# mache102/HashNeRF-pytorch

Hardware: AMD Instinct MI355X
Metric: training rays/sec (fwd+bwd) on chair; PSNR@5k iters (higher is better)
Workload: dtype fp32 (MLP GEMMs split-bf16 MFMA: 3 parts fwd, 2 parts grads); 1 GPU; chair 1xMI355X N_rand=4096 64+128 L16 F2 T19 finest512 (BASELINE configs[1]); rays_per_gpu=4096, global_batch=4096, samples_per_ray=64+128, log2_hashmap_size=19, finest_res=512, parallelism=dp1

## Files before the change

hashnerf-pytorch_amd/_lib.py:

```python
from __future__ import annotations

import ctypes as C
import os
from typing import Optional

import torch

HERE = os.path.dirname(os.path.abspath(__file__))
LIB_PATH = os.environ.get("HN_LIB_PATH") or os.path.join(HERE, "lib", "libhashnerf_amd.so")
MAX_LEVELS = 32
ABI_VERSION = 14
RENDER_FEAT_PER_RAY = 9728
MLP_PARAMS = 9344
MLP_PACKED_FLOATS = 30208

_lib = None


class HnGrid(C.Structure):
    _fields_ = [("n_levels", C.c_int32), ("n_features", C.c_int32),
                ("log2_hashmap_size", C.c_int32), ("reserved", C.c_int32),
                ("box_min", C.c_float * 3), ("box_max", C.c_float * 3),
                ("grid_size", (C.c_float * 3) * MAX_LEVELS)]

# ... 96 lines not shown
                ("g_raw_f", _P), ("d_table", _P), ("d_coarse", HnMlpGrad), ("d_fine", HnMlpGrad),
                ("table_step", C.POINTER(HnRadamTensor)), ("tv", C.c_void_p), ("g_tv", _P),
                ("table_live", _P), ("table_live_levels", C.c_int32), ("owner_defer", C.c_int32),
                ("loss", C.POINTER(HnRenderLoss)), ("mlp_step", C.POINTER(HnRadamTensor)),
                ("repack", C.c_int32), ("prepass_done", C.c_int32), ("next_batch", C.POINTER(HnNextBatch))]


class HnTvArgs(C.Structure):
    _fields_ = [("n_levels", C.c_int32), ("log2_hashmap_size", C.c_int32),
                ("cube", C.c_int32 * MAX_LEVELS), ("min_vertex", _P), ("table", _P)]


RADAM_MAX_TENSORS = 16


class HnRayPool(C.Structure):
    _fields_ = [("n_images", C.c_int32), ("H", C.c_int32), ("W", C.c_int32), ("pose_stride", C.c_int32),
                ("fx", C.c_double), ("fy", C.c_double), ("cx", C.c_double), ("cy", C.c_double),
                ("near", C.c_float), ("far", C.c_float), ("seed", C.c_uint64)]


POOL_ORDER_MAX = 8192

SIGNATURES = {
    "hn_abi_version": (C.c_int32, []),
    "hn_status_string": (C.c_char_p, [C.c_int32]),
    "hn_device_faults": (C.c_int32, [C.POINTER(C.c_int32), C.c_int32]),
    "hn_encode_fwd": (C.c_int32, [C.POINTER(HnGrid), _P, C.c_int64, _P, _P, _P, _P]),
    "hn_encode_bwd": (C.c_int32, [C.POINTER(HnGrid), _P, C.c_int64, _P, _P, _P]),
    "hn_sh_fwd": (C.c_int32, [_P, C.c_int64, _P, _P]),
    "hn_encode_bwd_input": (C.c_int32, [C.POINTER(HnGrid), _P, C.c_int64, _P, _P, _P, _P]),
    "hn_sh_bwd": (C.c_int32, [_P, _P, C.c_int64, _P, _P]),
    "hn_mlp_workspace_bytes": (C.c_size_t, []),
    "hn_mlp_fwd": (C.c_int32, [C.POINTER(HnMlp), _P, C.c_int64, _P, _P, C.c_size_t, _P]),
    "hn_mlp_bwd": (C.c_int32, [C.POINTER(HnMlp), _P, _P, C.c_int64, _P, C.POINTER(HnMlpGrad), _P,
                               C.c_size_t, _P]),
    "hn_composite_fwd": (C.c_int32, [_P, _P, _P, _P, C.c_int64, C.c_int32, C.c_int32, _P, _P, _P,
                                     _P, _P, _P, _P]),
    "hn_composite_bwd": (C.c_int32, [_P, _P, _P, _P, C.c_int64, C.c_int32, C.c_int32, _P, _P, _P,
                                     _P, _P, _P, _P]),
    "hn_composite_bwd_inputs": (C.c_int32, [_P, _P, _P, _P, C.c_int64, C.c_int32, C.c_int32, _P, _P, _P,
                                            _P, _P, _P, _P, _P]),
    "hn_sample_pdf": (C.c_int32, [_P, _P, _P, C.c_int64, C.c_int32, C.c_int32, _P, _P]),
    "hn_tv_fwd": (C.c_int32, [C.POINTER(HnTvArgs), _P, _P]),
    "hn_tv_bwd": (C.c_int32, [C.POINTER(HnTvArgs), _P, _P, _P]),
    "hn_radam_step": (C.c_int32, [C.POINTER(HnRadamTensor), C.c_int32, _P]),
    "hn_sample_rays": (C.c_int32, [C.POINTER(HnRaySampler), _P, _P, C.c_int64, _P, _P, _P]),
    "hn_sample_rays_morton_workspace_bytes": (C.c_size_t, [C.POINTER(HnRaySampler)]),
    "hn_uniform_philox": (C.c_int32, [C.c_uint64, C.POINTER(HnUniformDraw), C.c_int32, _P]),
    "hn_sample_batch_morton": (C.c_int32, [C.POINTER(HnRaySampler), _P, _P, C.c_int64, _P, _P, _P, C.c_size_t,
                                           C.c_uint64, C.POINTER(HnUniformDraw), C.c_int32, _P]),
    "hn_sample_rays_morton": (C.c_int32, [C.POINTER(HnRaySampler), _P, _P, C.c_int64, _P, _P, _P, C.c_size_t,
                                          _P]),
    "hn_sample_pool": (C.c_int32, [C.POINTER(HnRayPool), _P, _P, _P, C.c_int64, C.c_int64, _P, _P, _P]),
    "hn_sample_pool_ordered": (C.c_int32, [C.POINTER(HnRayPool), _P, _P, _P, C.c_int64, C.c_int64,
                                           C.POINTER(C.c_float), C.POINTER(C.c_float), _P, _P, _P, C.c_uint64,
                                           C.POINTER(HnUniformDraw), C.c_int32, _P]),
    "hn_sample_rays_ndc": (C.c_int32, [C.POINTER(HnRaySampler), _P, _P, C.c_int64, _P, _P, C.POINTER(HnRayNdc), _P]),
    "hn_sample_rays_morton_ndc": (C.c_int32, [C.POINTER(HnRaySampler), _P, _P, C.c_int64, _P, _P, _P, C.c_size_t,
                                              C.POINTER(HnRayNdc), _P]),
    "hn_sample_batch_morton_ndc": (C.c_int32, [C.POINTER(HnRaySampler), _P, _P, C.c_int64, _P, _P, _P, C.c_size_t,
                                               C.c_uint64, C.POINTER(HnUniformDraw), C.c_int32,
                                               C.POINTER(HnRayNdc), _P]),
    "hn_sample_pool_ndc": (C.c_int32, [C.POINTER(HnRayPool), _P, _P, _P, C.c_int64, C.c_int64, _P, _P,
                                       C.POINTER(HnRayNdc), _P]),
    "hn_sample_pool_ordered_ndc": (C.c_int32, [C.POINTER(HnRayPool), _P, _P, _P, C.c_int64, C.c_int64,
                                               C.POINTER(C.c_float), C.POINTER(C.c_float), _P, _P, _P, C.c_uint64,
                                               C.POINTER(HnUniformDraw), C.c_int32, C.POINTER(HnRayNdc), _P]),
    "hn_blender_images": (C.c_int32, [_P, C.c_int64, C.c_int32, C.c_int32, C.c_int32, C.c_int32, _P, _P]),
    "hn_loss_fwd": (C.c_int32, [_P, _P, _P, _P, _P, C.c_int64, _P, C.c_int32, C.c_float, C.c_float,
                                C.c_float, _P, _P]),
    "hn_loss_bwd": (C.c_int32, [_P, _P, _P, C.c_int64, C.c_int32, C.c_float, C.c_float, C.c_float, _P,
                                _P, _P, _P, _P, _P, _P]),
    "hn_loss_fwd_bwd": (C.c_int32, [_P, _P, _P, _P, _P, C.c_int64, _P, C.c_int32, C.c_float, C.c_float,
                                    C.c_float, _P, _P, _P, _P, _P, _P, _P, _P]),
    "hn_render_workspace_bytes": (C.c_size_t, [C.POINTER(HnRenderCfg), C.c_int64]),
    "hn_render_scatter_mode": (C.c_int32, [C.POINTER(HnRenderCfg), C.c_int64]),
    "hn_render_fwd": (C.c_int32, [C.POINTER(HnRenderCfg), C.POINTER(HnRenderFwdArgs), _P,
                                  C.c_size_t, _P]),
    "hn_render_fwd_form": (C.c_int32, [C.POINTER(HnRenderCfg), C.POINTER(HnRenderFwdArgs), C.c_int32, _P,
                                       C.c_size_t, _P]),
    "hn_render_fwd_pick": (C.c_int32, [C.c_int64, C.POINTER(C.c_int32)]),
    "hn_render_fwd_deal": (C.c_int32, [C.c_int64, C.c_int64, _P, _P]),
    "hn_render_bwd": (C.c_int32, [C.POINTER(HnRenderCfg), C.POINTER(HnRenderBwdArgs), _P,
                                  C.c_size_t, _P]),
    "hn_render_bwd_ndc": (C.c_int32, [C.POINTER(HnRenderCfg), C.POINTER(HnRenderBwdArgs), _P, C.c_size_t,
                                      C.POINTER(HnRayNdc), _P]),
    "hn_render_bwd_rays_workspace_bytes": (C.c_size_t, [C.POINTER(HnRenderCfg), C.c_int64]),
    "hn_render_bwd_rays": (C.c_int32, [C.POINTER(HnRenderCfg), C.POINTER(HnRenderBwdArgs), _P, C.c_size_t, _P, _P]),
    "hn_render_image_workspace_bytes": (C.c_size_t, [C.POINTER(HnRenderCfg)]),
    "hn_render_image": (C.c_int32, [C.POINTER(HnRenderCfg), C.POINTER(HnImageArgs), _P, C.c_size_t, _P]),
    "hn_render_image_variant": (C.c_int32, [C.POINTER(HnRenderCfg), C.POINTER(HnImageArgs), C.c_int32, _P,
                                            C.c_size_t, _P]),
    "hn_render_views_workspace_bytes": (C.c_size_t, [C.POINTER(HnRenderCfg)]),
    "hn_render_views": (C.c_int32, [C.POINTER(HnRenderCfg), C.POINTER(HnViewArgs), _P, C.c_size_t, _P]),
    "hn_render_bins": (C.c_int32, [C.POINTER(HnRenderCfg), C.c_int64, C.POINTER(C.c_int32)]),
    "hn_render_bwd_owner": (C.c_int32, [C.POINTER(HnRenderCfg), C.POINTER(HnRenderBwdArgs), _P,
                                        C.c_size_t, C.c_int32, C.c_int32, _P]),
}


def lib():
    global _lib
    if _lib is None:
        if not os.path.exists(LIB_PATH):
            raise RuntimeError(
                f"hashnerf_amd: HIP library not built ({LIB_PATH}); run "
                "`python -c 'import __graft_entry__ as g; g.build()'` -- there is no CPU fallback")
        L = C.CDLL(LIB_PATH)
        for name, (res, args) in SIGNATURES.items():
            fn = getattr(L, name)
            fn.restype = res
            fn.argtypes = args
        _lib = L
    return _lib


def check(status: int, what: str):
    if status != 0:
        msg = lib().hn_status_string(status).decode()
        raise RuntimeError(f"hashnerf_amd.{what} failed: {msg} (status {status})")


FAULT_BITS = {1: "ring slot wait", 2: "ring drain (tiles left unscattered)", 4: "coarse-grad flag wait",
              8: "dW buffer wait", 16: "binned-scatter overflow records exhausted",
              32: "non-finite (NaN / Inf) feature gradient or sample point in the binned scatter",
              64: "gradient on a table row pair the live mask marks dead (fused table step)",
              128: "prepass_done without a training forward of these rays on this workspace"}


def check_device_faults(clear: bool = True):
    w = C.c_int32(0)
    check(lib().hn_device_faults(C.byref(w), int(clear)), "device_faults")
    if w.value:
        what = ", ".join(v for k, v in FAULT_BITS.items() if w.value & k) or str(w.value)
        raise RuntimeError(f"hashnerf_amd: the render backward reported a fault ({what}); "
                           "the gradients of the launches since the last check are invalid")


def ptr(t: Optional[torch.Tensor]):
    return None if t is None else C.c_void_p(t.data_ptr())


def stream(device: torch.device):
    return C.c_void_p(torch.cuda.current_stream(device).cuda_stream)


def require_device(*tensors: torch.Tensor):
    for t in tensors:
        if t is None:
            continue
        if not t.is_cuda:
            raise RuntimeError("hashnerf_amd: tensors must live on a ROCm (HIP) device; "
                               "the reference CPU path is not part of this package")
        if t.dtype != torch.float32:
            raise TypeError(f"hashnerf_amd: expected float32, got {t.dtype}")


def contig(t: Optional[torch.Tensor]):
    return None if t is None else t.contiguous()


def make_grid(n_levels, n_features, log2T, box_min, box_max, grid_sizes) -> HnGrid:
    g = HnGrid()
    g.n_levels, g.n_features, g.log2_hashmap_size = int(n_levels), int(n_features), int(log2T)
    bmin = [float(v) for v in box_min]
# ... 23 lines not shown
```

hashnerf-pytorch_amd/csrc/hn_mlp.h:

```cpp
#pragma once
#include "hn_common.h"

namespace hn {

constexpr int kSplitF = 3;
constexpr int kSplitB = 2;
enum : int { R_F0, R_F1, R_F2G, R_F2S, R_F3, R_F4, R_B4, R_B3, R_B2G, R_B2S, R_B1, R_B0, R_N };
constexpr int kRegKS[R_N] = {16, 32, 8, 8, 32, 32, 4, 32, 32, 32, 8, 32};
constexpr int kRegOB[R_N] = {2, 1, 2, 2, 2, 1, 2, 2, 1, 1, 2, 1};
constexpr int kSplitFC = kSplitF;
constexpr int reg_ns(int r) {
  return kRegKS[r] % 8 ? 0 : (r < R_F2G ? kSplitF : (r < R_B4 ? kSplitFC : kSplitB));
}
constexpr int reg_gpo(int r) { return reg_ns(r) ? reg_ns(r) * kRegKS[r] / 8 : kRegKS[r] / 4; }
constexpr int reg_off(int r) {
  int o = 0;
  for (int i = 0; i < r; ++i) o += kRegOB[i] * reg_gpo(i) * 256;
  return o;
}
enum : int {
  G_F0 = reg_off(R_F0), G_F1 = reg_off(R_F1), G_F2G = reg_off(R_F2G), G_F2S = reg_off(R_F2S),
  G_F3 = reg_off(R_F3), G_F4 = reg_off(R_F4), G_B4 = reg_off(R_B4), G_B3 = reg_off(R_B3),
  G_B2G = reg_off(R_B2G), G_B2S = reg_off(R_B2S), G_B1 = reg_off(R_B1), G_B0 = reg_off(R_B0),
  G_END = reg_off(R_N)
};
static_assert(G_END <= HN_MLP_PACKED_FLOATS, "packed size");

enum : int { W_S0 = 0, W_S1 = 2048, W_C0 = 3072, W_C1 = 5056, W_C2 = 9152, W_END = 9344 };
static_assert(W_END == HN_MLP_PARAMS, "param count");

struct FragGlobal {
  static constexpr bool kRing = false;
  static constexpr int kLdsEnd = 0;
  const float* P;
  HN_DEV f32x4 operator()(int off, int lane) const { return frag_load(P, off, lane); }
};
struct FwdChunk {
  int r, ob, c;
};
constexpr FwdChunk kFwdSeq[] = {
    {R_F0, 0, 0}, {R_F0, 0, 1}, {R_F0, 1, 0}, {R_F0, 1, 1}, {R_F1, 0, 0}, {R_F1, 0, 1}, {R_F1, 0, 2},
    {R_F1, 0, 3}, {R_F2G, 0, 0}, {R_F2G, 1, 0}, {R_F3, 0, 0}, {R_F3, 0, 1}, {R_F3, 0, 2}, {R_F3, 0, 3},
    {R_F3, 1, 0}, {R_F3, 1, 1}, {R_F3, 1, 2}, {R_F3, 1, 3}, {R_F4, 0, 0}, {R_F4, 0, 1}, {R_F4, 0, 2},
    {R_F4, 0, 3}};
constexpr int kFwdSeqN = sizeof(kFwdSeq) / sizeof(kFwdSeq[0]);
constexpr int fwd_chunk_off(const FwdChunk& q) { return reg_off(q.r) + (q.ob * reg_gpo(q.r) + reg_ns(q.r) * q.c) * 256; }
constexpr int fwd_next_off(int r, int ob, int c) {
  for (int i = 0; i < kFwdSeqN; ++i)
    if (kFwdSeq[i].r == r && kFwdSeq[i].ob == ob && kFwdSeq[i].c == c) return fwd_chunk_off(kFwdSeq[(i + 1) % kFwdSeqN]);
  return -1;
}
struct FragRing {
  static constexpr bool kRing = true;
  static constexpr int kLdsEnd = 0;
  const float* P;
  float* slot;
  HN_DEV f32x4 operator()(int off, int lane) const { return frag_load(P, off, lane); }
};
constexpr int kFragResFloats = G_F2G;
struct FragRes {
  static constexpr bool kRing = false;
  static constexpr int kLdsEnd = kFragResFloats;
  const float* P;
  const float* res;
  HN_DEV f32x4 operator()(int off, int lane) const { return frag_load(P, off, lane); }
  HN_DEV f32x4 lds(int off, int lane) const { return *reinterpret_cast<const f32x4*>(res + off + 4 * lane); }
};
HN_DEV void ring_fill(const float* P, float* slot, int off, int lane) {
  int so = off * 4;
  asm volatile("" : "+s"(so));
  const __amdgpu_buffer_rsrc_t rs =
      __builtin_amdgcn_make_buffer_rsrc(const_cast<float*>(opaque_ptr(P)), (short)0, 0x7fffffff, 0x00020000);
#pragma unroll
  for (int q = 0; q < 3; ++q)
    __builtin_amdgcn_raw_ptr_buffer_load_lds(rs, (__attribute__((address_space(3))) void*)(slot + 256 * q), 16,
                                             lane * 16, so + 1024 * q, 0, 0);
}
HN_DEV void fwd_ring_start(const float* P, float* slot, int lane) {
  ring_fill(P, slot, fwd_chunk_off(kFwdSeq[0]), lane);
}
template <int R, typename BF, typename Src>
HN_DEV f32x16 gemm_src(const Src& src, int ob, f32x16 acc, int lane, BF bval);
template <int R, typename BF>
HN_DEV f32x16 gemm(const float* __restrict__ P, int ob, f32x16 acc, int lane, BF bval) {
  return gemm_src<R>(FragGlobal{P}, ob, acc, lane, bval);
}
template <int R, typename BF, typename Src>
HN_DEV f32x16 gemm_src(const Src& src, int ob, f32x16 acc, int lane, BF bval) {
  constexpr int KS = kRegKS[R], NS = reg_ns(R), GPO = reg_gpo(R), OFF = reg_off(R);
  auto ld = [&](int g) {
    if constexpr (OFF < Src::kLdsEnd) return src.lds(OFF + (ob * GPO + g) * 256, lane);
    else return src(OFF + (ob * GPO + g) * 256, lane);
  };
  if constexpr (NS > 0) {
#pragma unroll
    for (int c = 0; c < KS / 8; ++c) {
      SP<NS> a;
      if constexpr (Src::kRing && NS == 3) {
        asm volatile("s_waitcnt vmcnt(0)" ::: "memory");
#pragma unroll
        for (int q = 0; q < NS; ++q) a.p[q] = as_bf16x8(*reinterpret_cast<const f32x4*>(src.slot + 256 * q + 4 * lane));
        asm volatile("s_waitcnt lgkmcnt(0)" ::: "memory");
        ring_fill(src.P, src.slot, fwd_next_off(R, ob, c), lane);
      } else {
#pragma unroll
        for (int q = 0; q < NS; ++q) a.p[q] = as_bf16x8(ld(NS * c + q));
      }
      const SP<NS> b = splitn<NS>([&](int j) { return bval(8 * c + j); });
      acc = mfma_split<NS>(a, b, acc);
      __builtin_amdgcn_sched_barrier(0);
    }
    return acc;
  } else {
    f32x4 an = ld(0);
#pragma unroll
    for (int g = 0; g < KS / 4; ++g) {
      const f32x4 a = an;
      if (g + 1 < KS / 4) an = ld(g + 1);
#pragma unroll
      for (int j = 0; j < 4; ++j) acc = mfma(a[j], bval(4 * g + j), acc);
      __builtin_amdgcn_sched_barrier(0);
    }
    return acc;
  }
}

struct MlpAct {
  f32x16 h0[2];
  f32x16 s1;
  f32x16 c0[2];
  f32x16 c1[2];
  uint32_t m[3];
};
HN_DEV void relu_mask_or(const f32x16& v, uint32_t& m, int ob) {
  uint32_t w = 0u;
#pragma unroll
  for (int r = 15; r >= 0; --r) w = __builtin_amdgcn_alignbit(w, 0u - __float_as_uint(v[r]), 31u);
  m |= w << (16 * ob);
}

HN_DEV void relu16(f32x16& v) {
#pragma unroll
  for (int r = 0; r < 16; ++r) v[r] = __int_as_float(max(__float_as_int(v[r]), 0));
}
HN_DEV void mask16(f32x16& g, const f32x16& act) {
#pragma unroll
  for (int r = 0; r < 16; ++r) g[r] = act[r] > 0.f ? g[r] : 0.f;
}

struct NoLive {
  HN_DEV void operator()() const {}
};
template <bool MASKS = false, typename C0Init, typename Src, typename OnLive = NoLive>
HN_DEV void mlp_fwd_tile_src(const Src& P, const f32x16& feat, C0Init&& c0init, MlpAct& a, f32x16& c2,
                             int lane, bool skip_dead = false, OnLive&& on_live = OnLive{});
template <bool MASKS = false, typename C0Init>
HN_DEV void mlp_fwd_tile_c0(const float* __restrict__ P, const f32x16& feat, C0Init&& c0init,
                            MlpAct& a, f32x16& c2, int lane) {
  mlp_fwd_tile_src<MASKS>(FragGlobal{P}, feat, c0init, a, c2, lane);
}
template <bool MASKS, typename C0Init, typename Src, typename OnLive>
HN_DEV void mlp_fwd_tile_src(const Src& P, const f32x16& feat, C0Init&& c0init, MlpAct& a, f32x16& c2,
                             int lane, bool skip_dead, OnLive&& on_live) {
  a.m[0] = a.m[1] = a.m[2] = 0u;
#pragma unroll
  for (int ob = 0; ob < 2; ++ob) {
    a.h0[ob] = gemm_src<R_F0>(P, ob, zero16(), lane, [&](int s) { return feat[s]; });
    relu16(a.h0[ob]);
    if constexpr (MASKS) relu_mask_or(a.h0[ob], a.m[0], ob);
  }
  if constexpr (MASKS) asm volatile("" : "+v"(a.m[0]));
  a.s1 = gemm_src<R_F1>(P, 0, zero16(), lane, [&](int s) { return a.h0[s >> 4][s & 15]; });
  if (skip_dead && __ballot(lane < 32 && a.s1[0] > 0.f) == 0ull) {
    c2 = zero16();
    if constexpr (Src::kRing) {
      asm volatile("s_waitcnt vmcnt(0)" ::: "memory");
      ring_fill(P.P, P.slot, fwd_chunk_off(kFwdSeq[0]), lane);
    }
    return;
  }
  on_live();
#pragma unroll
  for (int ob = 0; ob < 2; ++ob) {
    f32x16 acc = c0init(ob);
    acc = gemm_src<R_F2G>(P, ob, acc, lane, [&](int s) { return a.s1[s]; });
    relu16(acc);
// ... 217 lines not shown
```

hashnerf-pytorch_amd/csrc/hn_render.hip:

```cpp
#include "hn_render_args.h"
#include "hn_render_fwd.h"
#include "hn_render_image.h"
#include "hn_mlp_bwd.h"
#include "hn_bwd_binned.h"
#include "hn_bwd_atomic.h"
#include "hn_bwd_rays.h"

#include <math.h>

#include <atomic>
#include <type_traits>

namespace hn {

__global__ __launch_bounds__(256) void render_comp_bwd_kernel(B1K k) {
  __shared__ float lds[kFwdWaves][kSf * 5];
  const int wave = __builtin_amdgcn_readfirstlane((int)threadIdx.x >> 6);
  const int lane = threadIdx.x & 63;
  if (k.bins && blockIdx.x == 0) zero_ovf_book(k);
  if (k.lout && blockIdx.x == 0) {
    loss_fwd_block<64 * kFwdWaves>(k.lrgb, k.lrgb0, k.ltarget, k.lsp, k.lsp0, k.B, k.ltv, k.n_tv, k.lworld,
                                   k.lsparse_w, k.ltv_w, k.lout);
    return;
  }
// ... 270 lines not shown
                          size_t ofs_c, size_t ofs_f, hipStream_t s, FieldK& f) {
  float *Pc = ws_at<float>(workspace, ofs_c), *Pf = ws_at<float>(workspace, ofs_f);
  if (int32_t st = weights_packed ? 0 : mlp_pack2_launch(&coarse, Pc, &fine, Pf, s)) return st;
  f = FieldK{make_grid_args(cfg->grid), cfg->white_bkgd, cfg->lindisp, t_vals, u, table, Pc, Pf};
  return HN_OK;
}

}

using namespace hn;

extern "C" size_t hn_render_workspace_bytes(const hn_render_cfg* cfg, int64_t n_rays) {
  return bwd_plan(cfg, n_rays).bytes();
}

extern "C" int32_t hn_render_scatter_mode(const hn_render_cfg* cfg, int64_t n_rays) {
  return bwd_mode(cfg, n_rays) == kModeSplit ? 2 : 1;
}

extern "C" int32_t hn_device_faults(int32_t* faults, int32_t clear) {
  if (!faults) return HN_E_NULL;
  int32_t st = hip_status(hipMemcpyFromSymbol(faults, HIP_SYMBOL(g_hn_fault), sizeof(int32_t)));
  if (st || !clear || *faults == 0) return st;
  const int32_t zero = 0;
  return hip_status(hipMemcpyToSymbol(HIP_SYMBOL(g_hn_fault), &zero, sizeof(int32_t)));
}

static int device_cus() {
  static std::atomic<int> cached[64];
  int dev = 0;
  if (hipGetDevice(&dev) != hipSuccess || dev < 0 || dev >= 64) return 0;
  int n = cached[dev].load(std::memory_order_relaxed);
  if (n == 0) {
    if (hipDeviceGetAttribute(&n, hipDeviceAttributeMultiprocessorCount, dev) != hipSuccess || n < 0) n = 0;
    cached[dev].store(n, std::memory_order_relaxed);
  }
  return n;
}
static int fwd_pick_form(int64_t n_rays, int cus) {
  return cus > 0 && (n_rays + kFwdResWaves - 1) / kFwdResWaves >= cus ? 2 : 1;
}
template <class F>
static void with_bool(bool b, F&& f) { b ? f(std::true_type{}) : f(std::false_type{}); }
static void launch_fwd(bool loss, bool ni64, bool res, int64_t n_rays, hipStream_t s, const RenderK& k) {
  const int bw = fwd_block_waves(res);
  const dim3 grid((unsigned)((n_rays + bw - 1) / bw)), block(64 * bw);
  with_bool(loss, [&](auto kLoss) {
    with_bool(ni64, [&](auto kNi64T) {
      with_bool(res, [&](auto kRes) {
        constexpr int ni = decltype(kNi64T)::value ? kNi64 : kNi;
        hipLaunchKernelGGL((render_fwd_kernel<decltype(kLoss)::value, ni, decltype(kRes)::value>), grid, block, 0, s,
                           k);
      });
    });
  });
}

extern "C" int32_t hn_render_fwd_pick(int64_t n_rays, int32_t* cus) {
  const int n = device_cus();
  if (cus) *cus = n;
  return fwd_pick_form(n_rays, n);
}

extern "C" int32_t hn_render_fwd_deal(int64_t n_rays, int64_t n_blocks, const uint8_t* run_key,
                                      int32_t* first_ray) {
  if (!first_ray) return HN_E_NULL;
  if (n_rays < 0 || n_blocks < 1 || n_blocks > (INT32_MAX / kFwdResWaves) || n_rays > n_blocks * kFwdResWaves)
    return HN_E_SHAPE;
  if (run_key)
    for (int64_t i = 0; i < n_blocks * kFwdResRuns; ++i)
      if (run_key[i] > kFwdResRunRays) return HN_E_SHAPE;
  for (int64_t b = 0; b < n_blocks; ++b) {
    const int x = (int)(b % kFwdResXcds);
    auto key_at = [&](int j) {
      const int64_t run = fwd_res_xcd_run(x, j);
      return run_key && run * kFwdResRunRays < n_rays ? (int)run_key[run] : 0;
    };
    for (int s = 0; s < kFwdResRuns; ++s)
      first_ray[b * kFwdResRuns + s] = (int32_t)(
          fwd_res_deal(n_blocks, b, s, [&](int nr, int pos) { return fwd_res_select(nr, pos, key_at); }) *
          kFwdResRunRays);
  }
  return HN_OK;
}

extern "C" int32_t hn_render_fwd(const hn_render_cfg* cfg, const hn_render_fwd_args* a,
                                 void* workspace, size_t ws_bytes, void* stream) {
  return hn_render_fwd_form(cfg, a, 0, workspace, ws_bytes, stream);
}

extern "C" int32_t hn_render_fwd_form(const hn_render_cfg* cfg, const hn_render_fwd_args* a, int32_t form,
                                      void* workspace, size_t ws_bytes, void* stream) {
  int32_t st = check_cfg(cfg);
  if (st) return st;
  if (form < 0 || form > 2) return HN_E_SHAPE;
  if (!a) return HN_E_NULL;
  if (a->n_rays < 0) return HN_E_SHAPE;
  if (a->n_rays == 0) return HN_OK;
  if (!a->rays || !a->t_vals || !a->u || !a->table || !mlp_ok(a->coarse) || !mlp_ok(a->fine))
    return HN_E_NULL;
  if (cfg->perturb && !a->t_rand) return HN_E_NULL;
  if (!a->rgb || !a->depth || !a->acc || !a->sparsity || !a->rgb0 || !a->depth0 || !a->acc0 ||
      !a->sparsity0 || !a->z_std || !a->z_coarse || !a->z_fine || !a->raw_c || !a->raw_f ||
      !a->fine_src)
    return HN_E_NULL;
  if (!workspace) return HN_E_NULL;
  const BwdPlan plan = bwd_plan(cfg, a->n_rays);
  if (ws_bytes < plan.bytes()) return HN_E_WORKSPACE;
  const bool ni64 = cfg->n_importance == kNi64;
  if (ni64 && a->feat && plan.mode != kModeSplit) return HN_E_SHAPE;
  if (a->loss) {
    if (!a->loss->target) return HN_E_NULL;
    if (!(a->loss->world > 0.f)) return HN_E_SHAPE;
    if (plan.mode != kModeSplit) return HN_E_SHAPE;
  }
  hipStream_t s = (hipStream_t)stream;
  RenderK k{};
  const WsLayout& L = plan.ws;
  if ((st = field_args(cfg, a->t_vals, a->u, a->table, a->coarse, a->fine, a->weights_packed, workspace, L.Pc, L.Pf,
                       s, k.f)))
    return st;
  k.perturb = cfg->perturb;
  k.B = a->n_rays;
  k.rays = a->rays; k.t_rand = a->t_rand;
  k.noise_c = a->noise_c; k.noise_f = a->noise_f;
  k.rgb = a->rgb; k.depth = a->depth; k.acc = a->acc; k.sparsity = a->sparsity;
  k.rgb0 = a->rgb0; k.depth0 = a->depth0; k.acc0 = a->acc0; k.sparsity0 = a->sparsity0;
  k.z_std = a->z_std; k.z_coarse = a->z_coarse; k.z_fine = a->z_fine;
  k.raw_c = a->raw_c; k.raw_f = a->raw_f; k.fine_src = a->fine_src; k.feat = a->feat;
  k.feat_nt = cfg->grid.log2_hashmap_size > 20;
  k.skip_dead = a->skip_dead_color != 0;
  const bool res = (form ? form : fwd_pick_form(a->n_rays, device_cus())) == 2;
  if (a->loss) {
    k.ltarget = a->loss->target;
    loss_factors(a->loss->world, a->loss->sparse_w, a->n_rays, k.lgm, k.lsparse);
    k.draw = ws_at<float>(workspace, L.draw);
    k.uflags = ws_at<uint8_t>(workspace, L.marks);
    k.stamp = ws_stamp(ws_at<int32_t>(workspace, L.lmeta));
  }
  launch_fwd(a->loss != nullptr, ni64, res, a->n_rays, s, k);
  return hip_status(hipGetLastError());
}

struct ImageWs {
  size_t Pc, Pf, slots, total;
};
static ImageWs image_ws_layout() {
  WsCursor c;
  ImageWs w;
  w.Pc = c.take(G_END);
  w.Pf = c.take(G_END);
  w.slots = c.take((size_t)kImgBlocks * kImgBlockWaves * kImgSlotFloats);
  w.total = c.at;
  return w;
}

extern "C" size_t hn_render_image_workspace_bytes(const hn_render_cfg* cfg) {
  return check_image_cfg(cfg) ? 0 : image_ws_layout().total * sizeof(float);
}
extern "C" size_t hn_render_views_workspace_bytes(const hn_render_cfg* cfg) {
  return check_cfg(cfg) ? 0 : image_ws_layout().total * sizeof(float);
}

static void launch_image(const hn_render_cfg* cfg, hipStream_t s, const ImageK& k) {
  const dim3 grid(kImgBlocks), block(64 * kImgBlockWaves);
  with_bool(cfg->n_importance == kNi64, [&](auto kNi64T) {
// ... 433 lines not shown
```

hashnerf-pytorch_amd/csrc/hn_render_fwd.h:

```cpp
#pragma once
#include "hn_render_args.h"

#define HN_FWD_PRIO_HI() __builtin_amdgcn_s_setprio(1)
#define HN_FWD_PRIO_LO() __builtin_amdgcn_s_setprio(0)

namespace hn {

constexpr int kFZc = 0, kFZsrc = 64, kFZs = 256, kFRaw = 448, kFW = 1216, kFBins = 1280,
              kFCdf = 1344, kFC0 = 1408, kFLds = 1472;

constexpr int kFwdWavesPerSimd = 4;

constexpr int kFwdBlockWaves = kFwdWaves;
constexpr int kFwdResWaves = 16;
constexpr int kFwdResRuns = 4;
constexpr int fwd_block_waves(bool res) { return res ? kFwdResWaves : kFwdBlockWaves; }

#ifndef HN_HOST_DEV
#define HN_HOST_DEV __host__ __device__ inline
#endif
constexpr int kFwdResRunRays = kFwdResWaves / kFwdResRuns;
constexpr int kFwdResSeg = 64;
constexpr int kFwdResSegRuns = kFwdResSeg / kFwdResRunRays;
constexpr int kFwdResXcds = 8;
// ... 25 lines not shown
  return 0;
}
template <class Select>
HN_HOST_DEV int64_t fwd_res_deal(int64_t nb, int64_t block, int s, Select&& select) {
  if (!fwd_res_deal_on(nb)) return fwd_res_band_run(nb, block, s);
  const int nw = (int)(nb / kFwdResXcds);
  return fwd_res_xcd_run((int)(block % kFwdResXcds),
                         select(fwd_res_xcd_runs(nb), fwd_res_deal_pos(nw, (int)(block / kFwdResXcds), s)));
}
HN_DEV int fwd_res_select_wave(const uint8_t* keys, int nr, int pos, int lane) {
  int cnt[kFwdResRunRays + 1] = {};
  for (int base = 0; base < nr; base += 64) {
    const int key = base + lane < nr ? (int)keys[base + lane] : -1;
#pragma unroll
    for (int b = 0; b <= kFwdResRunRays; ++b) cnt[b] += __popcll(__ballot(key == b));
  }
  int b = kFwdResRunRays;
#pragma unroll
  for (int t = kFwdResRunRays; t > 0; --t)
    if (b == t && pos >= cnt[t]) {
      pos -= cnt[t];
      b = t - 1;
    }
  if (cnt[b] == nr) return __builtin_amdgcn_readfirstlane(pos);
  int found = 0, seen = 0;
  for (int base = 0; base < nr; base += 64) {
    const bool mine = base + lane < nr && (int)keys[base + lane] == b;
    const uint64_t m = __ballot(mine);
    const int before = seen + (int)__builtin_amdgcn_mbcnt_hi((uint32_t)(m >> 32), __builtin_amdgcn_mbcnt_lo((uint32_t)m, 0u));
    const uint64_t hit = __ballot(mine && before == pos);
    if (hit) found = base + __builtin_ctzll(hit);
    seen += __popcll(m);
  }
  return __builtin_amdgcn_readfirstlane(found);
}


HN_DEV float coarse_z(float t, float near, float far, int lindisp) {
  return lindisp ? 1.f / (1.f / near * (1.f - t) + 1.f / far * t) : near * (1.f - t) + far * t;
}

template <bool kRes = false>
HN_DEV void pass_start(const float* P, const float sh8[8], float* L, float* ring, int lane, bool drain) {
  c0sh_lds_store(opaque_ptr(P), sh8, L + kFC0, lane);
  lds_fence_wave();
  if (drain) asm volatile("s_waitcnt vmcnt(0)" ::: "memory");
  if constexpr (!kRes) fwd_ring_start(P, ring, lane);
}

HN_DEV void load_twin_feat(const float* tiles, int src, int h, f32x16& feat) {
  const f32x4* t = reinterpret_cast<const f32x4*>(tiles + (size_t)(src >> 5) * 1024) + (src & 31) + 32 * h;
#pragma unroll
  for (int c = 0; c < 4; ++c) {
    const f32x4 v = t[64 * c];
    feat[4 * c] = v.x; feat[4 * c + 1] = v.y; feat[4 * c + 2] = v.z; feat[4 * c + 3] = v.w;
  }
}

template <int kNiT = kNi>
HN_DEV void importance_sort(float* L, const float* u, uint8_t* org, int lane) {
  static_assert(kNiT == kNi || kNiT == kNi64, "importance_sort: 128 or 64 importance samples");
  float* zsrc = L + kFZsrc;
  lds_fence_wave();
  sample_pdf_wave(L + kFBins, L + kFW + 1, kSc - 2, L + kFCdf, u, kNiT, zsrc + kSc, lane);
  lds_fence_wave();
  if constexpr (kNiT == kNi) {
    if (!merge_sort_z(zsrc, L + kFZs, L + kFRaw, lane, org)) rank_sort_wave(zsrc, L + kFZs, kSf, lane, org, kSc);
  } else {
    if (!merge_sort_z64(zsrc, L + kFZs, L + kFRaw, lane, org))
      rank_sort_wave(zsrc, L + kFZs, kSc + kNiT, lane, org, kSc);
  }
}

template <int kPass, class Pol, int kFineT = kSf, bool kRes = false>
HN_DEV void pass_tiles(const FieldK& f, const float* gsl, float* ring, float* L, const Ray& r, int lane, Pol& pol) {
  const int p = lane & 31, h = lane >> 5;
  for (int tau = 0; tau < (kPass ? kFineT : kSc) / 32; ++tau) {
    const float* P = opaque_ptr(kPass ? f.Pf : f.Pc);
    if constexpr (kPass && (kFineT != kSf || kRes)) {
      int zero = 0;
      asm volatile("" : "+s"(zero));
      gsl += zero;
    }
    const int q = 32 * tau + p;
    float pt[3];
    ray_point(r, L[(kPass ? kFZs : kFZc) + q], pt);
    f32x16 feat;
    const float* twins = kPass ? pol.twins() : nullptr;
    const int src = twins ? pol.origin(q) : 255;
    if (src >= kSc) {
      HN_FWD_PRIO_HI();
      encode_tile(f.g, gsl, f.table, pt, h, feat);
      HN_FWD_PRIO_LO();
    } else {
      load_twin_feat(twins, src, h, feat);
    }
    MlpAct a;
    f32x16 c2;
    const bool dead_skip = pol.skip_dead(kPass);
    bool stored = kPass == 0 || !dead_skip;
    if (stored) pol.save_feat(kPass, tau, lane, feat);
    using Src = std::conditional_t<kRes, FragRes, FragRing>;
    mlp_fwd_tile_src<Pol::kMasks>(Src{P, ring}, feat, [&](int ob) { return c0sh_lds_load(L + kFC0, ob, lane); },
                                  a, c2, lane, dead_skip, [&]() {
                                    if (!stored) pol.save_feat(kPass, tau, lane, feat);
                                    stored = true;
                                  });
    const float4 o4 = make_float4(c2[0], c2[1], c2[2], a.s1[0]);
    if (stored) pol.save_masks(kPass, tau, lane, a.m);
    if (h == 0) {
      *reinterpret_cast<float4*>(L + kFRaw + 4 * q) = o4;
      pol.save_raw(kPass, q, o4);
    }
  }
}

template <bool kLoss, int kSfT>
struct TrainTiles {
  static constexpr bool kMasks = true;
  const RenderK& k;
  int64_t ray;
  const uint8_t* srcl;
  HN_DEV const float* twins() const { return k.feat ? k.feat + (size_t)ray * HN_RENDER_FEAT_PER_RAY : nullptr; }
  HN_DEV int origin(int q) const { return kLoss ? (int)srcl[q] : (int)k.fine_src[ray * kSfT + q]; }
  HN_DEV bool skip_dead(int pass) const { return k.skip_dead && (pass ? k.noise_f : k.noise_c) == nullptr; }
  HN_DEV void save_feat(int pass, int tau, int lane, const f32x16& feat) const {
    if (k.feat) store_feat(k.feat, ray, pass * (kSc / 32) + tau, lane, feat, k.feat_nt != 0);
  }
  HN_DEV void save_masks(int pass, int tau, int lane, const uint32_t (&m)[3]) const {
    if (k.feat) store_masks(k.feat, ray, pass * (kSc / 32) + tau, lane, m, k.feat_nt != 0);
  }
  HN_DEV void save_raw(int pass, int q, const float4& o4) const {
    *reinterpret_cast<float4*>(pass ? k.raw_f + (ray * kSfT + q) * 4 : k.raw_c + (ray * kSc + q) * 4) = o4;
  }
};

template <bool kLoss, int N>
HN_DEV void composite_pass(const RenderK& k, int64_t ray, float* rawb, const float* z, const float* noise, int S,
                           float dnorm, float* wout, CompOut& o, int lane) {
  if constexpr (!kLoss) {
    composite_fwd<N>(rawb, z, noise, S, dnorm, k.f.white != 0, wout, o, lane);
  } else {
    const float target[3] = {k.ltarget[3 * ray], k.ltarget[3 * ray + 1], k.ltarget[3 * ray + 2]};
    CompSamples<N> cs;
    composite_samples<N>(rawb, z, noise, S, dnorm, cs, lane);
    CompTotals t;
    composite_totals<N>(cs, t);
    composite_fwd_out<N>(cs, t, k.f.white != 0, wout, o, lane);
    CompGrad g;
    loss_comp_grad(g, k.lgm, k.lsparse, o.rgb[0], o.rgb[1], o.rgb[2], target);
    composite_bwd_raw<N>(cs, t, k.f.white != 0, g, nullptr, nullptr, rawb, lane);
    lds_fence_wave();
  }
}

template <bool kLoss, int kNiT, bool kRes = false>
__global__ __launch_bounds__(64 * fwd_block_waves(kRes))
__attribute__((amdgpu_waves_per_eu(kFwdWavesPerSimd, kFwdWavesPerSimd)))
void render_fwd_kernel(RenderK k) {
  constexpr int kSfT = kSc + kNiT;
  constexpr int kBW = fwd_block_waves(kRes);
  __shared__ __attribute__((aligned(16))) float smem[kBW * kFLds + kGsLds];
  static_assert(2 * kFragResFloats % (4 * kFwdResWaves) == 0, "a whole dwordx4 share per wave");
  __shared__ __attribute__((aligned(16))) float fring[kBW][kRes ? 2 * kFragResFloats / kFwdResWaves : 768];
  const int wave = __builtin_amdgcn_readfirstlane((int)threadIdx.x >> 6);
  const int lane = threadIdx.x & 63;
  float* gsl = smem + kBW * kFLds;
  stage_grid_sizes(k.f.g, gsl);
  const int64_t nb = gridDim.x;
  __shared__ uint8_t dkeys[kRes && kLoss ? kFwdResMaxRuns : 4];
  const bool deal = kRes && kLoss && fwd_res_deal_on(nb);
  const int share = fwd_res_xcd_runs(nb) * kFwdResRunRays;
  const float bg = k.f.white ? 1.f : 0.f;
  auto load_targets = [&](int base, float (&t)[3]) {
    const int lr = base + lane;
    const int64_t ry = fwd_res_xcd_run((int)(blockIdx.x % kFwdResXcds), lr / kFwdResRunRays) * kFwdResRunRays +
                       lr % kFwdResRunRays;
#pragma unroll
    for (int c = 0; c < 3; ++c) t[c] = ry < k.B ? k.ltarget[3 * ry + c] : bg;
  };
  auto store_keys = [&](int base, const float (&t)[3]) {
    const bool live = fabsf(t[0] - bg) > 1.f / 512 || fabsf(t[1] - bg) > 1.f / 512 || fabsf(t[2] - bg) > 1.f / 512;
    const uint64_t m = __ballot(live);
    if (lane < 64 / kFwdResRunRays)
      dkeys[base / kFwdResRunRays + lane] =
          (uint8_t)__popcll((m >> (kFwdResRunRays * lane)) & ((1u << kFwdResRunRays) - 1));
  };
  float tg[3] = {bg, bg, bg};
  if constexpr (kRes && kLoss) {
    if (deal && 64 * wave < share) load_targets(64 * wave, tg);
  }
  if constexpr (kRes) {
    constexpr int kN4 = kFragResFloats / 4;
    const f32x4* srcc = reinterpret_cast<const f32x4*>(k.f.Pc);
    const f32x4* srcf = reinterpret_cast<const f32x4*>(k.f.Pf);
    f32x4* dst = reinterpret_cast<f32x4*>(&fring[0][0]);
#pragma unroll
    for (int i = 0; i < (2 * kN4 + 64 * kBW - 1) / (64 * kBW); ++i) {
      const int j = i * 64 * kBW + (int)threadIdx.x;
      if (j < 2 * kN4) dst[j] = j < kN4 ? srcc[j] : srcf[j - kN4];
    }
  }
  if constexpr (kRes && kLoss) {
    if (deal)
      for (int base = 64 * wave; base < share; base += 64 * kBW) {
        if (base != 64 * wave) load_targets(base, tg);
        store_keys(base, tg);
      }
  }
  __syncthreads();
  const int64_t grp = nb % 8 == 0 ? (blockIdx.x % 8) * (nb / 8) + blockIdx.x / 8 : blockIdx.x;
  int64_t ray = grp * kBW + wave;
  if constexpr (kRes) {
    constexpr int kW = kFwdResRunRays;
    const int s = wave / kW;
    const int64_t run = fwd_res_deal(nb, blockIdx.x, s, [&](int nr, int pos) {
      if constexpr (kLoss) return fwd_res_select_wave(dkeys, nr, pos, lane);
      else return pos;
    });
    ray = run * kW + wave % kW;
  }
  if constexpr (kLoss) {
    if (blockIdx.x == 0 && threadIdx.x == 0) *k.stamp = stamp_word(k.B);
  }
  if (ray >= k.B) return;
  float* L = smem + wave * kFLds;
  float* zc = L + kFZc;
  float* zsrc = L + kFZsrc;
  float* zs = L + kFZs;
  float* rawb = L + kFRaw;
  float* wts = L + kFW;
  Ray r;
  load_ray(k.rays, ray, r);
  float sh8[8];

  auto zlin = [&](int i) { return coarse_z(k.f.tvals[i], r.near, r.far, k.f.lindisp); };
  float z = zlin(lane);
  if (k.perturb) {
    const float zm = lane > 0 ? zlin(lane - 1) : z;
    const float zp = lane < kSc - 1 ? zlin(lane + 1) : z;
    const float lower = lane > 0 ? .5f * (z + zm) : z;
    const float upper = lane < kSc - 1 ? .5f * (zp + z) : z;
    z = lower + (upper - lower) * k.t_rand[ray * kSc + lane];
  }
  zc[lane] = z;
  zsrc[lane] = z;
  k.z_coarse[ray * kSc + lane] = z;
  ray_sh(r, lane >> 5, sh8);
  lds_fence_wave();

  uint8_t* srcl = reinterpret_cast<uint8_t*>(zsrc);
  TrainTiles<kLoss, kSfT> pol{k, ray, srcl};
  float* srcc = kRes ? &fring[0][0] : fring[wave];
  float* srcf = kRes ? &fring[0][0] + kFragResFloats : fring[wave];
  pass_start<kRes>(k.f.Pc, sh8, L, srcc, lane, false);
  pass_tiles<0, TrainTiles<kLoss, kSfT>, kSf, kRes>(k.f, gsl, srcc, L, r, lane, pol);
  lds_fence_wave();
  CompOut co;
  composite_pass<kLoss, kSc / 64>(k, ray, rawb, zc, k.noise_c ? k.noise_c + ray * kSc : nullptr, kSc, r.dnorm, wts,
                                  co, lane);
  if (lane == 0) {
#pragma unroll
    for (int c = 0; c < 3; ++c) k.rgb0[3 * ray + c] = co.rgb[c];
    k.depth0[ray] = co.depth;
    k.acc0[ray] = co.acc;
    k.sparsity0[ray] = co.entropy;
  }
  unsigned long long cmask = 0ull;
  if constexpr (kLoss) {
    const uint32_t nzu = draw_store_marks(rawb, k.draw + (size_t)ray * (kSc + kSf) * 4, kSc, lane);
    if (lane == 0) k.uflags[kMarkB * ray] = (uint8_t)nzu;
    cmask = coarse_nonzero_mask(rawb, lane);
  }

  if (lane < kSc - 1) L[kFBins + lane] = .5f * (zc[lane + 1] + zc[lane]);
  importance_sort<kNiT>(L, k.f.u + ray * kNiT, k.fine_src + ray * kSfT, lane);
  {
    if constexpr (kNiT == kNi) {
      const float s0 = zsrc[kSc + lane], s1 = zsrc[kSc + 64 + lane];
      const double mean = wave_sum((double)s0 + (double)s1) / kNi;
      const double d0 = (double)s0 - mean, d1 = (double)s1 - mean;
      const double var = wave_sum(d0 * d0 + d1 * d1) / kNi;
      if (lane == 0) k.z_std[ray] = (float)sqrt(var);
    } else {
      const double s0 = (double)zsrc[kSc + lane];
      const double d0 = s0 - wave_sum(s0) / kNiT;
      const double var = wave_sum(d0 * d0) / kNiT;
      if (lane == 0) k.z_std[ray] = (float)sqrt(var);
    }
  }
  for (int i = lane; i < kSfT; i += 64) k.z_fine[ray * kSfT + i] = zs[i];

  pass_start<kRes>(k.f.Pf, sh8, L, srcf, lane, true);
  if constexpr (kLoss) {
    for (int i = lane; i < kSfT; i += 64) srcl[i] = k.fine_src[ray * kSfT + i];
    lds_fence_wave();
  }
  pass_tiles<1, TrainTiles<kLoss, kSfT>, kSfT, kRes>(k.f, gsl, srcf, L, r, lane, pol);
  lds_fence_wave();
  CompOut fo;
  composite_pass<kLoss, kSfT / 64>(k, ray, rawb, zs, k.noise_f ? k.noise_f + ray * kSfT : nullptr, kSfT, r.dnorm,
                                   nullptr, fo, lane);
  if (lane == 0) {
#pragma unroll
    for (int c = 0; c < 3; ++c) k.rgb[3 * ray + c] = fo.rgb[c];
    k.depth[ray] = fo.depth;
    k.acc[ray] = fo.acc;
    k.sparsity[ray] = fo.entropy;
  }
  if constexpr (kLoss) {
    const uint32_t nzf = draw_store_marks(rawb, k.draw + ((size_t)ray * (kSc + kSf) + kSc) * 4, kSfT, lane);
    const uint32_t su = scatter_marks<kSfT>(rawb, srcl, cmask, lane);
    if (lane == 0) store_fine_marks(k.uflags, ray, nzf, su);
  }
}

}
```

include/hashnerf_amd.h:

```cpp
#ifndef HASHNERF_AMD_H
#define HASHNERF_AMD_H

#include <stddef.h>
#include <stdint.h>

#ifdef __cplusplus
extern "C" {
#endif

#define HN_ABI_VERSION 14
#define HN_MAX_LEVELS 32

enum {
  HN_OK = 0,
  HN_E_NULL = 1,
  HN_E_SHAPE = 2,
  HN_E_WORKSPACE = 3,
  HN_E_HIP = 1000
};

typedef struct hn_grid {
  int32_t n_levels;
  int32_t n_features;
  int32_t log2_hashmap_size;
// ... 180 lines not shown
  uint64_t offset;
} hn_uniform_draw;
#define HN_UNIFORM_MAX_DRAWS 4
int32_t hn_uniform_philox(uint64_t seed, const hn_uniform_draw* draws, int32_t n_draws, void* stream);
int32_t hn_sample_batch_morton(const hn_ray_sampler* s, const float* image, const float* c2w, int64_t n_rays,
                               float* rays, float* target, void* workspace, size_t ws_bytes, uint64_t seed,
                               const hn_uniform_draw* draws, int32_t n_draws, void* stream);

typedef struct hn_ray_ndc {
  float sx, sy;
} hn_ray_ndc;
int32_t hn_sample_rays_ndc(const hn_ray_sampler* s, const float* image, const float* c2w, int64_t n_rays,
                           float* rays, float* target, const hn_ray_ndc* ndc, void* stream);
int32_t hn_sample_rays_morton_ndc(const hn_ray_sampler* s, const float* image, const float* c2w, int64_t n_rays,
                                  float* rays, float* target, void* workspace, size_t ws_bytes,
                                  const hn_ray_ndc* ndc, void* stream);
int32_t hn_sample_batch_morton_ndc(const hn_ray_sampler* s, const float* image, const float* c2w, int64_t n_rays,
                                   float* rays, float* target, void* workspace, size_t ws_bytes, uint64_t seed,
                                   const hn_uniform_draw* draws, int32_t n_draws, const hn_ray_ndc* ndc,
                                   void* stream);

typedef struct hn_next_batch {
  const hn_ray_sampler* sampler;
  const float* image;
  const float* c2w;
  int64_t n_rays;
  float* rays;
  float* target;
  void* workspace;
  size_t ws_bytes;
  uint64_t seed;
  const hn_uniform_draw* draws;
  int32_t n_draws;
} hn_next_batch;
int32_t hn_render_bwd_ndc(const hn_render_cfg* cfg, const hn_render_bwd_args* a, void* workspace, size_t ws_bytes,
                          const hn_ray_ndc* next_ndc, void* stream);

typedef struct hn_ray_pool {
  int32_t n_images;
  int32_t H, W;
  int32_t pose_stride;
  double fx, fy, cx, cy;
  float near, far;
  uint64_t seed;
} hn_ray_pool;
int32_t hn_sample_pool(const hn_ray_pool* p, const float* images, const float* poses, const int32_t* image_ids,
                       int64_t start, int64_t n_rays, float* rays, float* target, void* stream);
#define HN_POOL_ORDER_MAX 8192
int32_t hn_sample_pool_ordered(const hn_ray_pool* p, const float* images, const float* poses,
                               const int32_t* image_ids, int64_t start, int64_t n_rays, const float* box_min,
                               const float* box_max, float* rays, float* target, uint32_t* keys, uint64_t seed,
                               const hn_uniform_draw* draws, int32_t n_draws, void* stream);
int32_t hn_sample_pool_ndc(const hn_ray_pool* p, const float* images, const float* poses, const int32_t* image_ids,
                           int64_t start, int64_t n_rays, float* rays, float* target, const hn_ray_ndc* ndc,
                           void* stream);
int32_t hn_sample_pool_ordered_ndc(const hn_ray_pool* p, const float* images, const float* poses,
                                   const int32_t* image_ids, int64_t start, int64_t n_rays, const float* box_min,
                                   const float* box_max, float* rays, float* target, uint32_t* keys, uint64_t seed,
                                   const hn_uniform_draw* draws, int32_t n_draws, const hn_ray_ndc* ndc,
                                   void* stream);

int32_t hn_blender_images(const uint8_t* rgba, int64_t n_images, int32_t H, int32_t W, int32_t half_res,
                          int32_t mode, float* out, void* stream);

int32_t hn_loss_fwd(const float* rgb, const float* rgb0, const float* target, const float* sp,
                    const float* sp0, int64_t n_rays, const float* tv, int32_t n_tv, float world,
                    float sparse_w, float tv_w, float* out, void* stream);
int32_t hn_loss_bwd(const float* rgb, const float* rgb0, const float* target, int64_t n_rays,
                    int32_t n_tv, float world, float sparse_w, float tv_w, const float* g_loss,
                    float* g_rgb, float* g_rgb0, float* g_sp, float* g_sp0, float* g_tv, void* stream);
int32_t hn_loss_fwd_bwd(const float* rgb, const float* rgb0, const float* target, const float* sp,
                        const float* sp0, int64_t n_rays, const float* tv, int32_t n_tv, float world,
                        float sparse_w, float tv_w, float* out, const float* g_loss, float* g_rgb,
                        float* g_rgb0, float* g_sp, float* g_sp0, float* g_tv, void* stream);

size_t hn_render_workspace_bytes(const hn_render_cfg* cfg, int64_t n_rays);
int32_t hn_render_scatter_mode(const hn_render_cfg* cfg, int64_t n_rays);
int32_t hn_render_fwd(const hn_render_cfg* cfg, const hn_render_fwd_args* a,
                      void* workspace, size_t ws_bytes, void* stream);
int32_t hn_render_fwd_form(const hn_render_cfg* cfg, const hn_render_fwd_args* a, int32_t form,
                           void* workspace, size_t ws_bytes, void* stream);
int32_t hn_render_fwd_pick(int64_t n_rays, int32_t* cus);
int32_t hn_render_fwd_deal(int64_t n_rays, int64_t n_blocks, const uint8_t* run_key, int32_t* first_ray);
int32_t hn_render_bwd(const hn_render_cfg* cfg, const hn_render_bwd_args* a,
                      void* workspace, size_t ws_bytes, void* stream);

size_t hn_render_bwd_rays_workspace_bytes(const hn_render_cfg* cfg, int64_t n_rays);
int32_t hn_render_bwd_rays(const hn_render_cfg* cfg, const hn_render_bwd_args* a, void* scratch, size_t bytes,
                           float* d_rays, void* stream);

typedef struct hn_image_args {
  int32_t n_views, H, W;
  int32_t pose_stride;
  float fx, fy, cx, cy;
  float near, far;
  const float* poses;
  const float* t_vals;
  const float* u;
  const float* table;
  hn_mlp coarse, fine;
  float* rgb;
  float* depth; float* acc;
  float* rays;
  int32_t weights_packed;
} hn_image_args;
size_t  hn_render_image_workspace_bytes(const hn_render_cfg* cfg);
int32_t hn_render_image(const hn_render_cfg* cfg, const hn_image_args* a, void* workspace, size_t ws_bytes,
                        void* stream);
int32_t hn_render_image_variant(const hn_render_cfg* cfg, const hn_image_args* a, int32_t variant,
                                void* workspace, size_t ws_bytes, void* stream);

typedef struct hn_view_args {
  hn_image_args image;
  int32_t ndc;
  float ndc_sx, ndc_sy;
  int32_t variant;
} hn_view_args;
size_t  hn_render_views_workspace_bytes(const hn_render_cfg* cfg);
int32_t hn_render_views(const hn_render_cfg* cfg, const hn_view_args* a, void* workspace, size_t ws_bytes,
                        void* stream);

#ifdef __cplusplus
}
#endif
#endif
```

Measured before the change: 8.435 million rays/s.

## Compact LDS-resident MLP weight image to hold F0,F1,F2G and trimmed F4 fragments

The LDS-resident weight image for the fused forward kernel used to cover only the leading regions up to F2G. It now uses a compacted layout that keeps only the useful lanes of each fragment group: half the lanes for F1, three for the small F4 output layer, and all of F0 and F2G. With that, the output layer also reads from LDS instead of global memory. A remap table gathers the image at kernel start, and a host export function exposes the mapping. The aim is fewer global fragment loads per tile, at the cost of masked lane reads, extra index arithmetic and a gather during block setup.

```diff
diff --git a/hashnerf-pytorch_amd/_lib.py b/hashnerf-pytorch_amd/_lib.py
--- a/hashnerf-pytorch_amd/_lib.py
+++ b/hashnerf-pytorch_amd/_lib.py
@@ -202,6 +202,7 @@
                                        C.c_size_t, _P]),
     "hn_render_fwd_pick": (C.c_int32, [C.c_int64, C.POINTER(C.c_int32)]),
     "hn_render_fwd_deal": (C.c_int32, [C.c_int64, C.c_int64, _P, _P]),
+    "hn_render_fwd_res_map": (C.c_int32, [C.c_int32, _P, C.c_int64, _P, C.c_int64]),
     "hn_render_bwd": (C.c_int32, [C.POINTER(HnRenderCfg), C.POINTER(HnRenderBwdArgs), _P,
                                   C.c_size_t, _P]),
     "hn_render_bwd_ndc": (C.c_int32, [C.POINTER(HnRenderCfg), C.POINTER(HnRenderBwdArgs), _P, C.c_size_t,
diff --git a/hashnerf-pytorch_amd/csrc/hn_mlp.h b/hashnerf-pytorch_amd/csrc/hn_mlp.h
--- a/hashnerf-pytorch_amd/csrc/hn_mlp.h
+++ b/hashnerf-pytorch_amd/csrc/hn_mlp.h
@@ -26,12 +26,47 @@
 };
 static_assert(G_END <= HN_MLP_PACKED_FLOATS, "packed size");
 
+constexpr int kResRegs[] = {R_F0, R_F1, R_F2G, R_F4};
+constexpr int kResRegN = sizeof(kResRegs) / sizeof(kResRegs[0]);
+constexpr bool res_held(int r) { return r == R_F0 || r == R_F1 || r == R_F2G || r == R_F4; }
+constexpr int res_keep(int r) { return r == R_F1 ? 16 : r == R_F4 ? 3 : 32; }
+constexpr int res_group_floats(int r) { return 8 * res_keep(r); }
+constexpr int res_reg_floats(int r) { return kRegOB[r] * reg_gpo(r) * res_group_floats(r); }
+constexpr int res_reg_off(int r) {
+  int o = 0;
+  for (int i = 0; i < kResRegN && kResRegs[i] != r; ++i) o += res_reg_floats(kResRegs[i]);
+  return o;
+}
+constexpr int kResNetFloats = res_reg_off(R_N);
+constexpr int kResImageFloats = 2 * kResNetFloats;
+constexpr bool res_paired(int r) { return res_keep(r) == 16; }
+constexpr int res_group_off(int r, int t) {
+  return res_reg_off(r) + (res_paired(r) ? (t >> 1) * 256 + (t & 1) * 64 : t * res_group_floats(r));
+}
+constexpr int res_lane_off(int r, int lane) {
+  return (lane & 31) >= res_keep(r) ? -1 : res_keep(r) == 3 ? 4 * ((lane >> 5) * 3 + (lane & 31)) : 4 * lane;
+}
+constexpr int res_at(int r, int t, int lane) {
+  return res_held(r) && res_lane_off(r, lane) >= 0 ? res_group_off(r, t) + res_lane_off(r, lane) : -1;
+}
+constexpr int res_src(int i) {
+  int r = kResRegs[0];
+  for (int k = 1; k < kResRegN; ++k)
+    if (i >= res_reg_off(kResRegs[k])) r = kResRegs[k];
+  const int rel = i - res_reg_off(r), gf = res_paired(r) ? 256 : res_group_floats(r), keep = res_keep(r);
+  const int w = rel % gf, l = w >> 2;
+  const int t = res_paired(r) ? 2 * (rel / gf) + ((l >> 4) & 1) : rel / gf;
+  const int lane = res_paired(r) ? (l & 15) + (l & 32) : 32 * (l / keep) + l % keep;
+  return reg_off(r) + t * 256 + 4 * lane + (w & 3);
+}
+static_assert(kResNetFloats * 4 == 25728 && res_reg_off(R_F4) * 4 == 24576, "the resident image's budget");
+
 enum : int { W_S0 = 0, W_S1 = 2048, W_C0 = 3072, W_C1 = 5056, W_C2 = 9152, W_END = 9344 };
 static_assert(W_END == HN_MLP_PARAMS, "param count");
 
 struct FragGlobal {
   static constexpr bool kRing = false;
-  static constexpr int kLdsEnd = 0;
+  static constexpr bool kRes = false;
   const float* P;
   HN_DEV f32x4 operator()(int off, int lane) const { return frag_load(P, off, lane); }
 };
@@ -52,19 +87,28 @@
 }
 struct FragRing {
   static constexpr bool kRing = true;
-  static constexpr int kLdsEnd = 0;
+  static constexpr bool kRes = false;
   const float* P;
   float* slot;
   HN_DEV f32x4 operator()(int off, int lane) const { return frag_load(P, off, lane); }
 };
-constexpr int kFragResFloats = G_F2G;
 struct FragRes {
   static constexpr bool kRing = false;
-  static constexpr int kLdsEnd = kFragResFloats;
+  static constexpr bool kRes = true;
   const float* P;
   const float* res;
   HN_DEV f32x4 operator()(int off, int lane) const { return frag_load(P, off, lane); }
-  HN_DEV f32x4 lds(int off, int lane) const { return *reinterpret_cast<const f32x4*>(res + off + 4 * lane); }
+  template <int R>
+  HN_DEV f32x4 lds(int t, int lane) const {
+    const float* g = res + res_group_off(R, t);
+    if constexpr (res_keep(R) == 32) {
+      return *reinterpret_cast<const f32x4*>(g + 4 * lane);
+    } else {
+      f32x4 v = {0.f, 0.f, 0.f, 0.f};
+      if ((lane & 31) < res_keep(R)) v = *reinterpret_cast<const f32x4*>(g + res_lane_off(R, lane));
+      return v;
+    }
+  }
 };
 HN_DEV void ring_fill(const float* P, float* slot, int off, int lane) {
   int so = off * 4;
@@ -88,10 +132,9 @@
 template <int R, typename BF, typename Src>
 HN_DEV f32x16 gemm_src(const Src& src, int ob, f32x16 acc, int lane, BF bval) {
   constexpr int KS = kRegKS[R], NS = reg_ns(R), GPO = reg_gpo(R), OFF = reg_off(R);
-  auto ld = [&](int g) {
-    if constexpr (OFF < Src::kLdsEnd) return src.lds(OFF + (ob * GPO + g) * 256, lane);
-    else return src(OFF + (ob * GPO + g) * 256, lane);
-  };
+  auto ld = [&](int g) { return src(OFF + (ob * GPO + g) * 256, lane); };
+  int rl = lane;
+  if constexpr (Src::kRes && res_keep(R) == 3) asm volatile("" : "+v"(rl));
   if constexpr (NS > 0) {
 #pragma unroll
     for (int c = 0; c < KS / 8; ++c) {
@@ -102,6 +145,9 @@
         for (int q = 0; q < NS; ++q) a.p[q] = as_bf16x8(*reinterpret_cast<const f32x4*>(src.slot + 256 * q + 4 * lane));
         asm volatile("s_waitcnt lgkmcnt(0)" ::: "memory");
         ring_fill(src.P, src.slot, fwd_next_off(R, ob, c), lane);
+      } else if constexpr (Src::kRes && res_held(R)) {
+#pragma unroll
+        for (int q = 0; q < NS; ++q) a.p[q] = as_bf16x8(src.template lds<R>(ob * GPO + NS * c + q, rl));
       } else {
 #pragma unroll
         for (int q = 0; q < NS; ++q) a.p[q] = as_bf16x8(ld(NS * c + q));
diff --git a/hashnerf-pytorch_amd/csrc/hn_render.hip b/hashnerf-pytorch_amd/csrc/hn_render.hip
--- a/hashnerf-pytorch_amd/csrc/hn_render.hip
+++ b/hashnerf-pytorch_amd/csrc/hn_render.hip
@@ -376,6 +376,19 @@
           kFwdResRunRays);
   }
   return HN_OK;
+}
+
+extern "C" int32_t hn_render_fwd_res_map(int32_t fine, int32_t* src, int64_t n_src, int32_t* at, int64_t n_at) {
+  if (fine < 0 || fine > 1) return -HN_E_SHAPE;
+  const int n = kResNetFloats;
+  if ((src && n_src < n) || (at && n_at < G_B4 / 4)) return -HN_E_SHAPE;
+  if (src)
+    for (int i = 0; i < n; ++i) src[i] = res_src(i);
+  if (at)
+    for (int r = R_F0; r < R_B4; ++r)
+      for (int t = 0; t < kRegOB[r] * reg_gpo(r); ++t)
+        for (int lane = 0; lane < 64; ++lane) at[reg_off(r) / 4 + t * 64 + lane] = res_at(r, t, lane);
+  return n;
 }
 
 extern "C" int32_t hn_render_fwd(const hn_render_cfg* cfg, const hn_render_fwd_args* a,
diff --git a/hashnerf-pytorch_amd/csrc/hn_render_fwd.h b/hashnerf-pytorch_amd/csrc/hn_render_fwd.h
--- a/hashnerf-pytorch_amd/csrc/hn_render_fwd.h
+++ b/hashnerf-pytorch_amd/csrc/hn_render_fwd.h
@@ -131,6 +131,13 @@
       asm volatile("" : "+s"(zero));
       gsl += zero;
     }
+    int lane_s = lane;
+    if constexpr (kRes) {
+      int zero = 0;
+      asm volatile("" : "+s"(zero));
+      ring += zero;
+      lane_s += zero;
+    }
     const int q = 32 * tau + p;
     float pt[3];
     ray_point(r, L[(kPass ? kFZs : kFZc) + q], pt);
@@ -139,7 +146,7 @@
     const int src = twins ? pol.origin(q) : 255;
     if (src >= kSc) {
       HN_FWD_PRIO_HI();
-      encode_tile(f.g, gsl, f.table, pt, h, feat);
+      encode_tile(f.g, gsl, f.table, pt, lane_s >> 5, feat);
       HN_FWD_PRIO_LO();
     } else {
       load_twin_feat(twins, src, h, feat);
@@ -148,18 +155,18 @@
     f32x16 c2;
     const bool dead_skip = pol.skip_dead(kPass);
     bool stored = kPass == 0 || !dead_skip;
-    if (stored) pol.save_feat(kPass, tau, lane, feat);
+    if (stored) pol.save_feat(kPass, tau, lane_s, feat);
     using Src = std::conditional_t<kRes, FragRes, FragRing>;
     mlp_fwd_tile_src<Pol::kMasks>(Src{P, ring}, feat, [&](int ob) { return c0sh_lds_load(L + kFC0, ob, lane); },
                                   a, c2, lane, dead_skip, [&]() {
-                                    if (!stored) pol.save_feat(kPass, tau, lane, feat);
+                                    if (!stored) pol.save_feat(kPass, tau, lane_s, feat);
                                     stored = true;
                                   });
     const float4 o4 = make_float4(c2[0], c2[1], c2[2], a.s1[0]);
-    if (stored) pol.save_masks(kPass, tau, lane, a.m);
+    if (stored) pol.save_masks(kPass, tau, lane_s, a.m);
     if (h == 0) {
       *reinterpret_cast<float4*>(L + kFRaw + 4 * q) = o4;
-      pol.save_raw(kPass, q, o4);
+      pol.save_raw(kPass, 32 * tau + (lane_s & 31), o4);
     }
   }
 }
@@ -210,8 +217,8 @@
   constexpr int kSfT = kSc + kNiT;
   constexpr int kBW = fwd_block_waves(kRes);
   __shared__ __attribute__((aligned(16))) float smem[kBW * kFLds + kGsLds];
-  static_assert(2 * kFragResFloats % (4 * kFwdResWaves) == 0, "a whole dwordx4 share per wave");
-  __shared__ __attribute__((aligned(16))) float fring[kBW][kRes ? 2 * kFragResFloats / kFwdResWaves : 768];
+  static_assert(kResImageFloats % (4 * kFwdResWaves) == 0, "a whole dwordx4 share per wave");
+  __shared__ __attribute__((aligned(16))) float fring[kBW][kRes ? kResImageFloats / kFwdResWaves : 768];
   const int wave = __builtin_amdgcn_readfirstlane((int)threadIdx.x >> 6);
   const int lane = threadIdx.x & 63;
   float* gsl = smem + kBW * kFLds;
@@ -240,14 +247,14 @@
     if (deal && 64 * wave < share) load_targets(64 * wave, tg);
   }
   if constexpr (kRes) {
-    constexpr int kN4 = kFragResFloats / 4;
+    constexpr int kN4 = kResImageFloats / 4, kC4 = kResNetFloats / 4;
     const f32x4* srcc = reinterpret_cast<const f32x4*>(k.f.Pc);
     const f32x4* srcf = reinterpret_cast<const f32x4*>(k.f.Pf);
     f32x4* dst = reinterpret_cast<f32x4*>(&fring[0][0]);
 #pragma unroll
-    for (int i = 0; i < (2 * kN4 + 64 * kBW - 1) / (64 * kBW); ++i) {
+    for (int i = 0; i < (kN4 + 64 * kBW - 1) / (64 * kBW); ++i) {
       const int j = i * 64 * kBW + (int)threadIdx.x;
-      if (j < 2 * kN4) dst[j] = j < kN4 ? srcc[j] : srcf[j - kN4];
+      if (j < kN4) dst[j] = (j < kC4 ? srcc : srcf)[res_src(4 * (j < kC4 ? j : j - kC4)) >> 2];
     }
   }
   if constexpr (kRes && kLoss) {
@@ -301,7 +308,7 @@
   uint8_t* srcl = reinterpret_cast<uint8_t*>(zsrc);
   TrainTiles<kLoss, kSfT> pol{k, ray, srcl};
   float* srcc = kRes ? &fring[0][0] : fring[wave];
-  float* srcf = kRes ? &fring[0][0] + kFragResFloats : fring[wave];
+  float* srcf = kRes ? &fring[0][0] + kResNetFloats : fring[wave];
   pass_start<kRes>(k.f.Pc, sh8, L, srcc, lane, false);
   pass_tiles<0, TrainTiles<kLoss, kSfT>, kSf, kRes>(k.f, gsl, srcc, L, r, lane, pol);
   lds_fence_wave();
diff --git a/include/hashnerf_amd.h b/include/hashnerf_amd.h
--- a/include/hashnerf_amd.h
+++ b/include/hashnerf_amd.h
@@ -286,6 +286,7 @@
                            void* workspace, size_t ws_bytes, void* stream);
 int32_t hn_render_fwd_pick(int64_t n_rays, int32_t* cus);
 int32_t hn_render_fwd_deal(int64_t n_rays, int64_t n_blocks, const uint8_t* run_key, int32_t* first_ray);
+int32_t hn_render_fwd_res_map(int32_t fine, int32_t* src, int64_t n_src, int32_t* at, int64_t n_at);
 int32_t hn_render_bwd(const hn_render_cfg* cfg, const hn_render_bwd_args* a,
                       void* workspace, size_t ws_bytes, void* stream);
 
```

Result: faster. 8.624 million rays/s, median of 6 (+2.2%).
